# rpng/R-VIO

Measured on AMD Instinct MI355X. Metric: camera frames/sec (KLT+RANSAC track, IMU propagate, MSCKF update, augment/compose), 200 feat / 10-clone window, higher is better.
Workload: dtype f64 (filter) / u8+i32+f32 (KLT); 1 GPU; cfgB: synthetic EuRoC-shaped 752x480 @20Hz, 200 features, 10-clone window, IMU 200 Hz, single stream, equalizer on (CLAHE 3.0, 5x5), corners from the device detector (GFTT + cornerSubPix); parallelism=single GPU

## Files before the change

### r-vio_amd/csrc/filter_kernels.hip

```cpp
#include <type_traits>
#include "rvio_dev.h"
#include "../../include/rvio_hip.h"
#include "solve9.hip"

#include "literal.h"
__device__ const double kChi2Dev[500] = {
#include "chi2_table.inc"
};

typedef double d4 __attribute__((ext_vector_type(4)));

__device__ __forceinline__ double fast_rcp(double v) {
    double y = __builtin_amdgcn_rcp(v);
    y = fma(fma(-v, y, 1.0), y, y);
    return fma(fma(-v, y, 1.0), y, y);
}
__device__ __forceinline__ void sincos_fast(double x, double* sp, double* cp) {
    if (!(fabs(x) < 1e5)) { sincos(x, sp, cp); return; }
    const double kf = rint(x * 6.36619772367581382433e-01);
    double r = fma(-kf, 1.57079632679489655800e+00, x);
    r = fma(-kf, 6.12323399573676603587e-17, r);
    const int q = (int)kf & 3;
    const double z = r * r;
    double ps = fma(z, 1.58969099521155010221e-10, -2.50507602534068634195e-08);
// ... 1739 lines not shown
#pragma unroll
        for (int q = 0; q < 4; ++q) out[q] = p1[q] - acc[q] + s2 * acc2[q];
        return out;
    };
    const d4 xij = xtile(I * 16, J * 16);
    d4 xji = xij;
    if (I != J) xji = xtile(J * 16, I * 16);
#pragma unroll
    for (int q = 0; q < 4; ++q) tl[wave][lk + 4 * q][li] = xji[q];
    __builtin_amdgcn_wave_barrier();
#pragma unroll
    for (int q = 0; q < 4; ++q) {
        const int rr = lk + 4 * q, row = I * 16 + rr, col = J * 16 + li;
        const double v = .5 * (xij[q] + tl[wave][li][rr]);
        if (row < d && col < d) {
            Pout[(size_t)row + (size_t)col * ld] = v;
            if (I != J) Pout[(size_t)col + (size_t)row * ld] = v;
        }
    }
}

#define JL_LS 61
#define JL_LDS_DOUBLES (3 * 60 * JL_LS + 8 * 16 * JL_LS + 16)
__global__ __launch_bounds__(256) void joseph_lds_kernel(DevCfg cfg, int n, const double* __restrict__ P, const double* __restrict__ W, const double* __restrict__ Ab,
                                                         double* __restrict__ Pout, FilterMeta* __restrict__ meta, const double* __restrict__ x, double* __restrict__ x_out,
                                                         const double* __restrict__ dx_scr, int n_pairs, int dx_nt) {
    if (dx_scr && (int)blockIdx.x >= n_pairs) {
        __shared__ S9DxLds dxl;
        s9_dx_role(cfg, meta, n, Ab, x, P, dx_scr, x_out, dx_nt, (int)blockIdx.x - n_pairs, dxl);
        return;
    }
    extern __shared__ __align__(16) double jl[];
    constexpr int LS = JL_LS;
    double* const Wl = jl;
    double* const Al = Wl + 60 * LS;
    double* const Ccl = Al + 60 * LS;
    double* const PcS = Ccl + 60 * LS;
    double* const Us = PcS + 2 * 16 * LS;
    double* const Gs = Us + 2 * 16 * LS;
    double* const Qs = Gs + 2 * 16 * LS;
    constexpr int SS = 16 * LS;
    const int c6 = 6 * n, d = 24 + c6, ldh = cfg.ldh, ld = cfg.dmax;
    const double s2 = cfg.sigma_im * cfg.sigma_im;
    const int tid = threadIdx.x, lane = tid & 63, wave = tid >> 6, li = lane & 15, lk = lane >> 4;
    DBG_R(blockIdx.x == 0, 3);
    const int nt = (d + 15) / 16;
    int I = 0, rem = blockIdx.x;
    while (rem >= nt - I) { rem -= nt - I; ++I; }
    const int J = I + rem;
    const int r0[2] = {I * 16, J * 16};
    auto r0of = [&](int sidx) { return sidx ? J * 16 : I * 16; };
    DBG_T(20);
    double p0[4] = {0, 0, 0, 0}, p0t[4] = {0, 0, 0, 0};
    if (wave == 0) {
#pragma unroll
// ... 105 lines not shown
        for (int q = 0; q < 4; ++q) {
            if (wave < nprod) xt[wave][lk + 4 * q][li] = pa[q];
            if (two) xt[wave + 4][lk + 4 * q][li] = pb[q];
        }
    }
    __syncthreads();
    DBG_T(25);
    if (wave == 0) {
        const int o = (I == J) ? 0 : 3;
#pragma unroll
        for (int q = 0; q < 4; ++q) {
            const int rr = lk + 4 * q, row = I * 16 + rr, col = J * 16 + li;
            const double p1 = p0[q] - xt[0][rr][li];
            const double xij = p1 - xt[1][rr][li] + s2 * xt[2][rr][li];
            const double p1t = p0t[q] - xt[o][li][rr];
            const double xji = p1t - xt[o + 1][li][rr] + s2 * xt[o + 2][li][rr];
            const double v = .5 * (xij + xji);
            if (row < d && col < d) {
                Pout[(size_t)row + (size_t)col * ld] = v;
                if (I != J) Pout[(size_t)col + (size_t)row * ld] = v;
            }
        }
    }
}
```

### r-vio_amd/csrc/filter_kernels2.hip

```cpp
#pragma once
#include "rvio_dev.h"
#include "solve9.hip"

__device__ __forceinline__ double skew_e(const double* v, int i, int j) {
    if (i == j) return 0.0;
    const double e = v[3 - i - j];
    return (j == (i + 1) % 3) ? -e : e;
}

struct Prop3Sample { double dR[9], up[3], uv[3], w[3], dt, Rk[9], vk[3], gk[3]; };

template <int PROP3_CH>
struct Prop3Lds {
    double Pl[24][25];
    double Psi[24][25];
    double PhiSx[2][PROP3_CH][9][25];
    double PsiC[9][25];
    double Nq[PROP3_CH][9][6];
    double Qd[PROP3_CH][6][6];
    double vxs[PROP3_CH][9];
    Prop3Sample sm[PROP3_CH];
    double xs[26];
    double chain[9 + 3 * 5 + 1];
};
// ... 259 lines not shown
__global__ __launch_bounds__(256) void feat_prop_kernel(DevCfg cfg, int n, double* x, double* P,
                                                        const int* n_feat_ptr, const unsigned char* types, const int* lens, const float* meas,
                                                        double* Gshare, int* nrows_out, int* acc_out, int* ndof_out, double* gamma_out,
                                                        double* pfinv_out, double* tm_global, BatchIn bin,
                                                        FilterMeta* meta, const rvio_imu* imu, int m, double* chol_scr, int chol_nt, int shard_rank, int shard_world,
                                                        double* lit_rows) {
    DBG_R(blockIdx.x == 0, 0);
    DBG_W(blockIdx.x == 0 && threadIdx.x == 0, 28);
    extern __shared__ __align__(16) double fp_dyn[];
    if (blockIdx.x == gridDim.x - 1) { propagate_body<16>(cfg, meta, n, x, P, imu, m, 0, 0, *reinterpret_cast<Prop3Lds<16>*>(fp_dyn)); return; }
    if (chol_scr && blockIdx.x == gridDim.x - 2) {
        if (chol_nt == 4) s9_chol_role<2>(cfg, n, P, chol_scr, *reinterpret_cast<S9CholLds<4, 4>*>(fp_dyn));
        else s9_chol_role<3>(cfg, n, P, chol_scr, *reinterpret_cast<S9CholLds<6, 4>*>(fp_dyn));
        return;
    }
    feat_build_body<16>(cfg, n, x, P, n_feat_ptr, types, lens, meas, shard_rank, shard_world, Gshare, nrows_out, acc_out, ndof_out, gamma_out, pfinv_out, tm_global, 0, bin, meta, (int)blockIdx.x, nullptr, nullptr, lit_rows);
}

__device__ __forceinline__ int aug_src2(int a, int n, int nmax, int do_aug) {
    if (a < 24 || !do_aug) return a;
    const int cb = (a - 24) / 6, off = (a - 24) % 6;
    if (n < nmax) return (cb < n) ? a : 9 + off;
    return (cb < nmax - 1) ? a + 6 : 9 + off;
}
__global__ __launch_bounds__(256) void augcomp_kernel2(DevCfg cfg, int n, int do_aug, const double* __restrict__ x, const double* __restrict__ P,
                                                       double* __restrict__ x_out, double* __restrict__ P_out, double* __restrict__ pose_out, size_t bs,
                                                       unsigned long long* done) {
    DBG_R(blockIdx.x == 0, 5);
    x = zoff(x, bs); P = zoff(P, bs); x_out = zoff(x_out, bs); P_out = zoff(P_out, bs); pose_out = zoff(pose_out, bs);
    __shared__ double Vk[24][25];
    __shared__ double P11[24][25];
    __shared__ double Tm[24][25];
    __shared__ double xs[26];
    __shared__ double xo[17];
    const int nmax = cfg.nmax, ld = cfg.dmax;
    const int n2 = do_aug ? ((n < nmax) ? n + 1 : nmax) : n;
    const int d2 = 24 + 6 * n2, xd2 = 26 + 7 * n2;
    const int tid = threadIdx.x;
    if (tid < 26) xs[tid] = x[tid];
    for (int e = tid; e < 576; e += 256) Vk[e / 24][e % 24] = 0.0;
    const int gstride = ((int)gridDim.x - 1) * 256, e0 = ((int)blockIdx.x - 1) * 256 + tid, total = d2 * d2;
    double xv = 0.0, pr[9];
    bool pre = false;
    if (blockIdx.x == 0) {
        for (int e = tid; e < 576; e += 256) P11[e % 24][e / 24] = P[(size_t)(e % 24) + (size_t)(e / 24) * ld];
        static_assert(26 + 7 * (RVIO_MAX_LEN - 1) <= 256, "the state copy is one value per thread");
// ... 5 lines not shown
                else src = (cb < nmax - 1) ? i + 7 : 10 + off;
            }
            xv = x[src];
        }
    } else {
        for (int e = e0; e < total; e += gstride) {
            const int a = e % d2, b = e / d2;
            if (a < 24 && b < 24) continue;
            if (a >= 24 && b >= 24) { P_out[(size_t)a + (size_t)b * ld] = P[(size_t)aug_src2(a, n, nmax, do_aug) + (size_t)aug_src2(b, n, nmax, do_aug) * ld]; continue; }
            const int i = (a < 24) ? a : b;
            const double* pc = P + (size_t)aug_src2((a < 24) ? b : a, n, nmax, do_aug) * ld;
            if (i >= 15) P_out[(size_t)a + (size_t)b * ld] = pc[i];
            else if (i >= 9) P_out[(size_t)a + (size_t)b * ld] = 0.0;
            else if (e == e0) {
                const int b3 = 3 * (i / 3);
                pr[0] = pc[b3]; pr[1] = pc[b3 + 1]; pr[2] = pc[b3 + 2];
#pragma unroll
                for (int k = 0; k < 6; ++k) pr[3 + k] = pc[9 + k];
                pre = true;
            }
        }
    }
    __syncthreads();
    if (tid < 64) {
        const q4 qG = ldq(xs), qk = ldq(xs + 10);
        const d3 pG = ld3(xs + 4), pk = ld3(xs + 14);
        const m33 Rk = q2r(qk);
        const d3 gk = unit3(mv33(Rk, ld3(xs + 7)));
        const d3 pkG = mv33(Rk, sub3(pG, pk));
        if (tid == 0) {
            const m33 spx = skew33(pkG), sgx = skew33(gk);
#pragma unroll
            for (int i = 0; i < 3; ++i)
#pragma unroll
                for (int j = 0; j < 3; ++j) {
                    Vk[i][j] = Rk.m[3 * i + j];           Vk[i][9 + j] = (i == j) ? 1.0 : 0.0;
                    Vk[3 + i][3 + j] = Rk.m[3 * i + j];   Vk[3 + i][9 + j] = spx.m[3 * i + j];   Vk[3 + i][12 + j] = -Rk.m[3 * i + j];
                    Vk[6 + i][6 + j] = Rk.m[3 * i + j];   Vk[6 + i][9 + j] = sgx.m[3 * i + j];
                }
#pragma unroll
            for (int i = 15; i < 24; ++i) Vk[i][i] = 1.0;
            if (blockIdx.x == 0) {
                const q4 qkG = qmul(qk, qG);
                stq(xo, qkG); st3(xo + 4, pkG); st3(xo + 7, gk);
                xo[10] = 0; xo[11] = 0; xo[12] = 0; xo[13] = 1; xo[14] = 0; xo[15] = 0; xo[16] = 0;
                const d3 pGk = mv33(tr33(q2r(qG)), sub3(pk, pG));
                st3(pose_out, pGk); stq(pose_out + 3, qkG);
            }
        }
    }
    __syncthreads();
    if (blockIdx.x == 0) {
        for (int e = tid; e < 576; e += 256) {
            const int i = e / 24, j = e % 24;
            double a = 0;
            if (i >= 15) a = P11[i][j];
            else if (i < 9) {
                const int b3 = 3 * (i / 3);
#pragma unroll
                for (int k = 0; k < 3; ++k) a += Vk[i][b3 + k] * P11[b3 + k][j];
#pragma unroll
                for (int k = 9; k < 15; ++k) a += Vk[i][k] * P11[k][j];
            }
            Tm[i][j] = a;
        }
        __syncthreads();
        for (int e = tid; e < 576; e += 256) {
            const int i = e / 24, j = e % 24;
            double a = 0;
            if (j >= 15) a = Tm[i][j];
            else if (j < 9) {
                const int b3 = 3 * (j / 3);
#pragma unroll
                for (int k = 0; k < 3; ++k) a += Tm[i][b3 + k] * Vk[j][b3 + k];
#pragma unroll
                for (int k = 9; k < 15; ++k) a += Tm[i][k] * Vk[j][k];
            }
            P11[i][j] = a;
        }
        __syncthreads();
        for (int e = tid; e < 576; e += 256) { int i = e / 24, j = e % 24; P_out[(size_t)i + (size_t)j * ld] = .5 * (P11[i][j] + P11[j][i]); }
        for (int i = tid; i < xd2; i += 256) x_out[i] = (i < 17) ? xo[i] : xv;
    } else {
        for (int e = e0; e < total; e += gstride) {
            const int a = e % d2, b = e / d2;
            if ((a < 24) == (b < 24)) continue;
            const int i = (a < 24) ? a : b;
            if (i >= 9) continue;
            const int b3 = 3 * (i / 3);
            if (!(pre && e == e0)) {
                const double* pc = P + (size_t)aug_src2((a < 24) ? b : a, n, nmax, do_aug) * ld;
                pr[0] = pc[b3]; pr[1] = pc[b3 + 1]; pr[2] = pc[b3 + 2];
#pragma unroll
                for (int k = 0; k < 6; ++k) pr[3 + k] = pc[9 + k];
            }
            double acc = Vk[i][b3] * pr[0] + Vk[i][b3 + 1] * pr[1] + Vk[i][b3 + 2] * pr[2];
            acc += Vk[i][9] * pr[3] + Vk[i][10] * pr[4] + Vk[i][11] * pr[5];
            if (b3 == 3) acc += Vk[i][12] * pr[6] + Vk[i][13] * pr[7] + Vk[i][14] * pr[8];
            P_out[(size_t)a + (size_t)b * ld] = acc;
        }
    }
    DBG_R(blockIdx.x == 0, 6);
    if (done) stage_signal(done);
}
```

### r-vio_amd/csrc/rvio_hip.hip

```cpp
#include <hip/hip_runtime.h>
#include <atomic>
#include <chrono>
#include <dlfcn.h>
#include <cmath>
#include <cstdio>
#include <cstdlib>
#include <cstring>
#include <map>
#include <mutex>
#include <string>
#include <vector>

#include "../../include/rvio_hip.h"
#include "rvio_dev.h"
#include "frontend_dev.h"
#include "filter_kernels.hip"
#include "filter_kernels2.hip"
#include "solve6.hip"
#include "solve7.hip"
#include "solve9.hip"
#include "landmarks.hip"
#pragma clang fp contract(off)
#include "frontend_kernels.hip"
#include "klt3.hip"
// ... 6 lines not shown
    rvio_config cfg;
    DevCfg dc;
    int device = 0;
    hipStream_t stream = nullptr;
    hipStream_t stream_t = nullptr;
    hipStream_t ts = nullptr;
    hipEvent_t evT[4] = {nullptr, nullptr, nullptr, nullptr};
    hipEvent_t evH[4] = {nullptr, nullptr, nullptr, nullptr};
    static const int kHand = 4;
    hipEvent_t evF[kHand] = {nullptr, nullptr, nullptr, nullptr}, evIn[2] = {nullptr, nullptr};
    long frame_no = 0;
    bool piped = false, in_frame = false;
    struct TrackOut { int* n_feat; unsigned char* types; int* len; float* meas; } tout[kHand];
    std::string err;
    FilterMeta* meta = nullptr;
    double* x[2] = {nullptr, nullptr};
    double* P[2] = {nullptr, nullptr};
    int cur = 0;
    int img_count = 0;
    int n_clones_host = 0;
    double *partial = nullptr, *block = nullptr, *Ab = nullptr, *Tbuf = nullptr, *W = nullptr, *Mg = nullptr, *U = nullptr, *G = nullptr,
           *Pt1 = nullptr, *tm_global = nullptr, *gamma = nullptr, *pfinv = nullptr;
    int *nrows = nullptr, *acc = nullptr, *ndof = nullptr, *gram_cnt = nullptr;
    double* gpose = nullptr;
    int* gvalid = nullptr;
    size_t trunc_lds = 0, gram_batch_lds = 0;
    double *lit_rows = nullptr, *lit_state = nullptr;
    bool lit_state_global = false;
    size_t lit_batch_lds = 0;
    const double* last_Ab = nullptr;
    int feat_threads = 64;
    size_t feat_lds = 0, fprop_lds = 0, ug_lds = 0, book_lds = 0, jb_lds = 0;
    int book_waves = 4;
    bool book_fused = true;
    int solve5_variant = 0;
    StageSync* stage_sync = nullptr;
    StageSync stage_tgt = {};
    const unsigned long long* klt_wait = nullptr; unsigned long long klt_target = 0;
    unsigned long long* pyr_signal = nullptr;
    int solve7_variant = 0;
    int solve9_nt = 0;
    double* S9scr = nullptr;
    bool chol_ready = false;
    float* eig_map = nullptr;
    size_t solve5_lds = 0, cholt_lds = 0;
    rvio_imu* d_imu = nullptr;
    double* gathered = nullptr;
    int gathered_world = 0;
    int imu_cap = RVIO_MAX_IMU;
    float* d_cand = nullptr;
    uint8_t* d_img = nullptr;
    static const int kIC = 3;
    DetDev dets[kIC] = {};
    int det_set_last = 0;
    bool det_ready = false, use_det = false;
    hipStream_t stream_l = nullptr;
    hipEvent_t evA = nullptr, evL = nullptr;
    bool dx_pending = false;
    bool chol_async = false;
    hipStream_t stream_d = nullptr;
    hipStream_t stream_c = nullptr;
    hipEvent_t evC[kIC] = {nullptr, nullptr, nullptr};
    int n_ic = 2;
    int ic = 0;
    hipStream_t side = nullptr;
    hipEvent_t evD0 = nullptr, evD1 = nullptr;
    uint8_t* hb_img[2] = {nullptr, nullptr};
    rvio_imu* hb_imu[kHand + 1] = {nullptr, nullptr, nullptr, nullptr, nullptr};
    hipEvent_t book_wait = nullptr;
    int fin_mode[kHand] = {0, 0, 0, 0};
    unsigned long long fin_target[kHand] = {0, 0, 0, 0}, book_target = 0;
    bool book_dev = false;
    bool handover_evt = false;
    bool last_ra = false;
    float* hb_cand[2] = {nullptr, nullptr};
    static const int kPin = 3;
    uint8_t* pin[kPin] = {nullptr, nullptr, nullptr};
    hipEvent_t evPin[kPin] = {nullptr, nullptr, nullptr}, evPin2[kPin] = {nullptr, nullptr, nullptr};
    size_t pin_img = 0, pin_imu = 0, pin_bytes = 0;
    uint8_t *d_eq = nullptr, *d_lut2[kIC] = {nullptr, nullptr, nullptr};
// ... 149 lines not shown
    d->block_x = c->block_x; d->block_y = c->block_y;
    d->grid_cols = (int)std::floor(c->width / c->block_x);
    d->grid_rows = (int)std::floor(c->height / c->block_y);
    d->off_x = (float)(int)(.5 * (c->width - d->grid_cols * c->block_x));
    d->off_y = (float)(int)(.5 * (c->height - d->grid_rows * c->block_y));
    d->max_per_block = (d->grid_cols * d->grid_rows > 0) ? (float)(int)((float)c->n_features / (d->grid_cols * d->grid_rows)) : 0.f;
    d->use_sampson = c->use_sampson;
    d->fisheye = c->fisheye ? 1 : 0;
    int w = c->width, hgt = c->height, lv = 1;
    for (int l = 1; l <= 3; ++l) { w = (w + 1) / 2; hgt = (hgt + 1) / 2; if (w <= 15 || hgt <= 15) break; lv++; }
    d->levels = lv;
}

static int alloc_filter_slab(rvio_hip* h, bool need_tm_global) {
    const DevCfg& d = h->dc;
    const size_t dm = d.dmax, PP = dm * dm, ldh = d.ldh;
    TrackerDev& t = h->t;
    DALLOC(h, h->meta, 1);
    for (int b = 0; b < 2; ++b) { DALLOC(h, h->x[b], (size_t)d.xdmax + 8); DALLOC(h, h->P[b], PP); }
    DALLOC(h, h->partial, (size_t)d.Fu * ldh * ldh);
    DALLOC(h, h->block, 2 * ldh * ldh);
    DALLOC(h, h->Ab, 2 * ldh * ldh);
    DALLOC(h, h->gram_cnt, 8);
    DALLOC(h, h->stage_sync, 1);
    DALLOC(h, h->Tbuf, ldh * ldh); DALLOC(h, h->W, ldh * ldh);
    DALLOC(h, h->U, dm * ldh); DALLOC(h, h->G, dm * ldh);
    DALLOC(h, h->Pt1, PP);
    DALLOC(h, h->gamma, d.Fu); DALLOC(h, h->pfinv, (size_t)3 * d.Fu);
    DALLOC(h, h->nrows, d.Fu); DALLOC(h, h->acc, d.Fu); DALLOC(h, h->ndof, d.Fu);
    DALLOC(h, h->d_imu, RVIO_MAX_IMU);
    DALLOC(h, h->d_info, 1); DALLOC(h, h->d_pose, 8);
    DALLOC(h, t.n_feat, 1); DALLOC(h, t.types, d.Fu); DALLOC(h, t.len, d.Fu); DALLOC(h, t.meas, (size_t)2 * d.Fu * d.max_len);
    if (need_tm_global) DALLOC(h, h->tm_global, (size_t)d.Fu * d.rho_max * ldh);
    static const bool no_lit = getenv("RVIO_NO_LITERAL") != nullptr;
    if (!no_lit && d.ldh <= 190 && d.nmax + 1 <= 40 && d.rho_max < 254 && lit_slab_doubles(d.ldh, d.rho_max) * sizeof(double) <= 144 * 1024) {
        DALLOC(h, h->lit_rows, lit_rows_doubles(d.ldh, d.rho_max));
        if (h->lit_state_global) DALLOC(h, h->lit_state, lit_state_doubles(d.ldh - 1));
    }
    if (h->batch > 1 && d.max_len <= GEOM4_ML) { DALLOC(h, h->gpose, (size_t)d.Fu * (d.max_len - 1) * 24); DALLOC(h, h->gvalid, d.Fu); }
    return RVIO_OK;
}

static int detector_alloc(rvio_hip* h);
static int detector_check(rvio_hip* h);
static int alloc_frontend_slab(rvio_hip* h) {
    const DevCfg& d = h->dc;
// ... 51 lines not shown
    return e && *e && std::strcmp(e, "0") != 0 && std::strcmp(e, "False") != 0 && std::strcmp(e, "false") != 0;
}
static bool no_device_polls() {
    static const bool v = (paranoid_bits() & PAR_NO_DEVPOLL) || profiler_serialises();
    return v;
}

static hipError_t lds_attr(const void* fn, int bytes) {
    static std::mutex mu;
    static std::map<const void*, int> limit;
    std::lock_guard<std::mutex> lk(mu);
    int& cur = limit[fn];
    if (bytes <= cur) return hipSuccess;
    const hipError_t e = hipFuncSetAttribute(fn, hipFuncAttributeMaxDynamicSharedMemorySize, bytes);
    if (e == hipSuccess) cur = bytes;
    return e;
}
static_assert(LP_S9CHOL4_BYTES == sizeof(S9CholLds<4, 4>), "launch_plan.h: solve9's LDS structs");
static_assert(LP_S9CHOL6_BYTES == sizeof(S9CholLds<6, 4>), "launch_plan.h: solve9's LDS structs");
static_assert(LP_S9SMALL_BYTES == sizeof(S9SmallLds), "launch_plan.h: solve9's LDS structs");
static_assert(LP_PROP3_BYTES == sizeof(Prop3Lds<16>), "launch_plan.h: propagate's LDS struct");
static_assert(LP_JB_TL_DOUBLES == JB_TL_DOUBLES && LP_UGL_BYTES == UGL_LDS_DOUBLES * sizeof(double) && LP_FNL_BYTES == FNL_LDS_DOUBLES * sizeof(double) &&
              LP_JL_BYTES == JL_LDS_DOUBLES * sizeof(double), "launch_plan.h: the Joseph-form kernels' LDS");
static const void* lp_kernel_fn(int k) {
    switch (k) {
        case LPK_FEAT_BUILD16: return (const void*)feat_build_kernel<16>;
        case LPK_FEAT_BUILD4: return (const void*)feat_build_kernel<4>;
        case LPK_GRAM_REDUCE: return (const void*)gram_reduce_kernel;
        case LPK_BLOCK_SUM: return (const void*)block_sum_kernel;
        case LPK_LIT_BATCH: return (const void*)lit_batch_kernel;
        case LPK_GEMM_T_LDS: return (const void*)gemm_T_lds_kernel;
        case LPK_GRAM_BATCH4: return (const void*)gram_reduce_batch_kernel<4>;
        case LPK_GRAM_BATCH6: return (const void*)gram_reduce_batch_kernel<6>;
        case LPK_FEAT_PROP: return (const void*)feat_prop_kernel;
        case LPK_BOOKKEEP_B: return (const void*)bookkeep_b_kernel;
        case LPK_RANSAC_BOOK: return (const void*)ransac_book_kernel;
        case LPK_SOLVE9_SMALL: return (const void*)solve9_small_kernel;
        case LPK_SOLVE6_1: return (const void*)solve6_kernel<1, 8, 8>;
        case LPK_SOLVE6_2: return (const void*)solve6_kernel<2, 12, 8>;
        case LPK_SOLVE6_3: return (const void*)solve6_kernel<2, 16, 8>;
        case LPK_JOSEPH_BATCH: return (const void*)joseph_batch_kernel;
        case LPK_UG: return (const void*)ug_kernel;
        case LPK_UG_LDS: return (const void*)ug_lds_kernel;
        case LPK_FINAL_LDS: return (const void*)final_lds_kernel;
        case LPK_JOSEPH_LDS: return (const void*)joseph_lds_kernel;
    }
// ... 434 lines not shown
        return;
    }
    if (h->solve7_variant == 4)
        hipLaunchKernelGGL((solve7_kernel<3, 16, 12>), gb, dim3(768), 0, h->stream, d, h->meta, n, Ab, xin, Pc, h->Tbuf, h->W, xout, h->slab_bytes);
    else if (h->solve5_variant == 1)
        hipLaunchKernelGGL((solve6_kernel<1, 8, 8>), gb, dim3(512), h->solve5_lds, h->stream, d, h->meta, n, h->Tbuf, Ab, xin, Pc, h->W, xout, h->slab_bytes);
    else if (h->solve5_variant == 2)
        hipLaunchKernelGGL((solve6_kernel<2, 12, 8>), gb, dim3(512), h->solve5_lds, h->stream, d, h->meta, n, h->Tbuf, Ab, xin, Pc, h->W, xout, h->slab_bytes);
    else if (h->solve5_variant == 3)
        hipLaunchKernelGGL((solve6_kernel<2, 16, 8>), gb, dim3(512), h->solve5_lds, h->stream, d, h->meta, n, h->Tbuf, Ab, xin, Pc, h->W, xout, h->slab_bytes);
}

static void launch_ug_final(rvio_hip* h, int n, const double* Ab, double* Pn, bool ug, bool fin) {
    const DevCfg& d = h->dc;
    const int c6 = 6 * n, dd = 24 + c6, B = h->batch;
    const size_t bs = h->slab_bytes;
    double* Pc = h->P[h->cur];
    const int nt = (dd + 15) / 16, npair = nt * (nt + 1) / 2;
    if (h->jb_lds && ug && fin) {
        hipLaunchKernelGGL(joseph_batch_kernel, dim3(1, 1, B), dim3(JB_THREADS), h->jb_lds, h->stream, d, n, Pc, h->W, Ab, Pn, bs);
    } else if (B == 1 && c6 <= 60 && ug && fin) {
        const bool dxr = h->dx_pending;
        h->dx_pending = false;
        hipLaunchKernelGGL(joseph_lds_kernel, dim3(npair + (dxr ? (dd + 23) / 24 : 0)), dim3(256), JL_LDS_DOUBLES * sizeof(double), h->stream, d, n, Pc, h->W, Ab, Pn,
                           h->meta, (const double*)h->x[h->cur], h->x[h->cur ^ 1], dxr ? (const double*)h->S9scr : (const double*)nullptr, npair, h->solve9_nt);
    } else if (B == 1 && c6 <= 64) {
        if (ug) hipLaunchKernelGGL(ug_lds_kernel, dim3(nt), dim3(256), UGL_LDS_DOUBLES * sizeof(double), h->stream, d, n, Pc, h->W, Ab, h->U, h->G, h->Pt1);
        if (fin) hipLaunchKernelGGL(final_lds_kernel, dim3((npair + 3) / 4), dim3(256), FNL_LDS_DOUBLES * sizeof(double), h->stream, d, n, h->Pt1, h->G, h->U, Pn);
    } else if (B == 1) {
        const int c6t = (c6 + 15) / 16;
        if (ug) {
            const bool dxr = h->dx_pending;
            h->dx_pending = false;
            const double* nod = nullptr;
            hipLaunchKernelGGL(ug_tile_kernel<0>, dim3((nt * c6t + 3) / 4 + (dxr ? (dd + 23) / 24 : 0)), dim3(256), 0, h->stream, d, n, Pc, h->W, Ab, h->U, h->G, h->Pt1,
                               h->meta, (const double*)h->x[h->cur], h->x[h->cur ^ 1], dxr ? (const double*)h->S9scr : nod, h->solve9_nt);
            hipLaunchKernelGGL(ug_tile_kernel<1>, dim3((nt * c6t + 3) / 4), dim3(256), 0, h->stream, d, n, Pc, h->W, Ab, h->U, h->G, h->Pt1, h->meta, nod, (double*)nullptr, nod, 0);
            hipLaunchKernelGGL(ug_tile_kernel<2>, dim3((nt * nt + 3) / 4), dim3(256), 0, h->stream, d, n, Pc, h->W, Ab, h->U, h->G, h->Pt1, h->meta, nod, (double*)nullptr, nod, 0);
        }
        if (fin) hipLaunchKernelGGL(final_tile_kernel, dim3(npair), dim3(256), 0, h->stream, d, n, h->Pt1, h->G, h->U, Pn);
    } else {
        if (ug) hipLaunchKernelGGL(ug_kernel, dim3((dd + 15) / 16, 1, B), dim3(256), h->ug_lds, h->stream, d, n, Pc, h->W, Ab, h->U, h->G, h->Pt1, bs);
        if (fin) hipLaunchKernelGGL(final_kernel, dim3((npair + 3) / 4, 1, B), dim3(256), 0, h->stream, d, n, h->Pt1, h->G, h->U, Pn, bs);
    }
}

static void launch_landmarks(rvio_hip* h, int n, const LmOut& out) {
    const int T = std::min(LM_MAX_T, 64 * ((h->dc.Fu + 63) / 64));
// ... 126 lines not shown
    SYNC_FRONT(h);
    HIPCHK(h, hipStreamSynchronize(h->stream));
    const size_t o = (size_t)instance * h->lm.bs;
    int cnt = 0;
    if (h->lm_frame >= 0) {
        HIPCHK(h, hipMemcpyAsync(&cnt, (char*)h->lm.count + o, sizeof cnt, hipMemcpyDeviceToHost, h->stream));
        HIPCHK(h, hipStreamSynchronize(h->stream));
        cnt = std::max(0, std::min(cnt, h->dc.Fu));
    }
    if (n) *n = cnt;
    if (frame) *frame = h->lm_frame;
    if (cnt > 0) {
        if (feat) HIPCHK(h, hipMemcpyAsync(feat, (char*)h->lm.feat + o, sizeof(int) * cnt, hipMemcpyDeviceToHost, h->stream));
        if (p_r) HIPCHK(h, hipMemcpyAsync(p_r, (char*)h->lm.p_r + o, sizeof(double) * 3 * cnt, hipMemcpyDeviceToHost, h->stream));
        if (p_world) HIPCHK(h, hipMemcpyAsync(p_world, (char*)h->lm.p_w + o, sizeof(double) * 3 * cnt, hipMemcpyDeviceToHost, h->stream));
        HIPCHK(h, hipStreamSynchronize(h->stream));
    }
    return RVIO_OK;
}
int rvio_hip_get_landmarks(rvio_hip* h, int32_t* n, int32_t* frame, int32_t* feat, double* p_r, double* p_world) {
    return rvio_hip_get_landmarks_at(h, 0, n, frame, feat, p_r, p_world);
}

static int augment_compose_dev(rvio_hip* h, int do_augment) {
    const DevCfg& d = h->dc;
    const int c = h->cur, o = c ^ 1;
    const int cg = 1 + (h->batch >= 128 ? 4 : std::max(1, std::min(64, (d.dmax * d.dmax + 255) / 256)));
    unsigned long long* done = nullptr;
    if (h->batch == 1) { done = &h->stage_sync->aug; h->stage_tgt.aug += (unsigned long long)cg; }
    if (h->chol_async) { HIPCHK(h, hipStreamWaitEvent(h->stream, h->evL, 0)); h->chol_async = false; }
    hipLaunchKernelGGL(augcomp_kernel2, dim3(cg, 1, h->batch), dim3(256), 0, h->stream, d, h->n_clones_host, do_augment, h->x[c], h->P[c], h->x[o], h->P[o], h->d_pose,
                       h->slab_bytes, done);
    HIPCHK(h, hipGetLastError());
    h->cur = o;
    h->chol_ready = false;
    if (do_augment && h->n_clones_host < d.nmax) h->n_clones_host++;
    if (h->solve9_nt >= 8 && h->stream_l && !profiler_serialises() && h->n_clones_host >= 1) {
        HIPCHK(h, hipEventRecord(h->evA, h->stream));
        HIPCHK(h, hipStreamWaitEvent(h->stream_l, h->evA, 0));
        if (h->solve9_nt == 8) hipLaunchKernelGGL((solve9_chol_kernel<2, 4>), dim3(1), dim3(1024), 0, h->stream_l, d, h->n_clones_host, h->P[h->cur], h->S9scr);
        else hipLaunchKernelGGL((solve9_chol_kernel<3, 4>), dim3(1), dim3(1024), 0, h->stream_l, d, h->n_clones_host, h->P[h->cur], h->S9scr);
        HIPCHK(h, hipEventRecord(h->evL, h->stream_l));
        h->chol_async = true;
    }
    return RVIO_OK;
}
int rvio_hip_augment_compose(rvio_hip* h, int do_augment) {
    if (!h) return RVIO_ERR_INVALID;
    HIPCHK(h, hipSetDevice(h->device));
    return augment_compose_dev(h, do_augment);
}

static int detector_check(rvio_hip* h) {
    const int cell1 = (int)std::nearbyint((double)h->cfg.min_dist);
    if (cell1 < 1) { h->err = "Tracker.nMinDist < 1 is not supported by the device detector"; return RVIO_ERR_UNSUPPORTED; }
    const int spw = (int)std::floor(.5 * h->cfg.min_dist);
    if (spw < 1 || spw > 63) { h->err = "device cornerSubPix takes half-windows 1..63 (2 <= Tracker.nMinDist < 128)"; return RVIO_ERR_UNSUPPORTED; }
    return RVIO_OK;
}
static int detector_alloc_set(rvio_hip* h, DetDev& q) {
    const DevCfg& d = h->dc;
    const int cell1 = (int)std::nearbyint((double)h->cfg.min_dist), cell2 = (int)std::nearbyint((double)(2.f * h->cfg.min_dist));
    const size_t npx = (size_t)d.W * d.H;
    q.W = d.W; q.H = d.H; q.F = d.F; q.min_dist = h->cfg.min_dist; q.quality = (double)h->cfg.qual_lvl;
    q.max_cells = ((d.W + cell1 - 1) / cell1) * ((d.H + cell1 - 1) / cell1);
    q.first = h->t.first;
    q.eig = nullptr;
    DALLOC(h, q.maxkey, 1); DALLOC(h, q.counters, 4); DALLOC(h, q.cell_cnt, (size_t)q.max_cells);
// ... 316 lines not shown

int rvio_hip_frame_plan(rvio_hip* h, int* do_update, int* do_augment) {
    if (!h) return RVIO_ERR_INVALID;
    h->img_count++;
    if (do_update) *do_update = (h->n_clones_host > h->cfg.min_track_len - 1) ? 1 : 0;
    if (do_augment) *do_augment = (h->img_count > 1) ? 1 : 0;
    return RVIO_OK;
}
int rvio_hip_propagate_dev(rvio_hip* h, const rvio_imu* d_imu, int m) {
    if (!h || (!d_imu && m > 0) || m < 0) return RVIO_ERR_INVALID;
    HIPCHK(h, hipSetDevice(h->device));
    return propagate_dev(h, d_imu, m);
}

static int wait_filter_done(rvio_hip* h, int b, hipStream_t stream) {
    if (h->fin_mode[b] == 0) HIPCHK(h, hipStreamWaitEvent(stream, h->evF[b], 0));
    else HIPCHK(h, hipStreamSynchronize(h->stream));
    return RVIO_OK;
}
static int frame_tail_dev(rvio_hip* h, const rvio_imu* d_imu, int m, bool propagated = false) {
    h->img_count++;
    int rc = propagated ? RVIO_OK : propagate_dev(h, d_imu, m);
    if (rc != RVIO_OK) return rc;
    if (h->n_clones_host > h->cfg.min_track_len - 1) {
        rc = rvio_hip_update_tracked(h);
        if (rc != RVIO_OK) return rc;
    }
    return augment_compose_dev(h, h->img_count > 1);
}
int rvio_hip_frame_tracks_dev(rvio_hip* h, const rvio_imu* d_imu, int imu_stride, int m, const int32_t* d_n_feat, const unsigned char* d_types,
                              const int32_t* d_len, const float* d_meas) {
    if (!h || (!d_imu && m > 0) || m < 0 || imu_stride < 0 || (imu_stride > 0 && imu_stride < m)) return RVIO_ERR_INVALID;
    if (!d_n_feat || !d_types || !d_len || !d_meas) return RVIO_ERR_INVALID;
    if (h->piped || h->in_frame) { h->err = "rvio_hip_frame_tracks_dev on a handle that runs the pipelined image path"; return RVIO_ERR_INVALID; }
    HIPCHK(h, hipSetDevice(h->device));
    const DevCfg& d = h->dc;
    h->img_count++;
    const bool upd = h->n_clones_host > h->cfg.min_track_len - 1;
    const bool overlap = upd && h->batch > 1 && !h->front_end;
    int rc;
    if (overlap) {
        HIPCHK(h, hipEventRecord(h->evD0, h->stream));
        HIPCHK(h, hipStreamWaitEvent(h->stream_t, h->evD0, 0));
        rc = propagate_dev(h, d_imu, m, (size_t)imu_stride * sizeof(rvio_imu), h->stream_t);
        HIPCHK(h, hipEventRecord(h->evD1, h->stream_t));
    } else rc = propagate_dev(h, d_imu, m, (size_t)imu_stride * sizeof(rvio_imu));
    if (rc != RVIO_OK) return rc;
    if (upd) {
        const TrackerDev t0 = h->t;
        const BatchIn b0 = h->bin;
        h->t.n_feat = const_cast<int*>(d_n_feat); h->t.types = const_cast<unsigned char*>(d_types);
// ... 564 lines not shown
```

Before: 11060 frames/s.

## Fuse augment/compose into Joseph update kernel via last-block tail

Runs the augment/compose step as a tail inside joseph_lds_kernel: the last block to finish, detected with an atomic counter, builds Vk, rotates the 24x24 core block, transforms the cross-covariance columns and copies the clone block. This drops a separate augcomp_kernel2 launch and its dependency gap on the single-stream update path. The cost is that the whole augment runs serially in one 256-thread block rather than spread over many blocks. The host tracks the fused state and adjusts the stage-sync target to match.

```diff
diff --git a/r-vio_amd/csrc/filter_kernels.hip b/r-vio_amd/csrc/filter_kernels.hip
--- a/r-vio_amd/csrc/filter_kernels.hip
+++ b/r-vio_amd/csrc/filter_kernels.hip
@@ -1785,15 +1785,25 @@
 
 #define JL_LS 61
 #define JL_LDS_DOUBLES (3 * 60 * JL_LS + 8 * 16 * JL_LS + 16)
+struct AugTail { int on, do_aug; double* x_dst; double* P_dst; double* pose_out; int* cnt; unsigned long long* done; };
+__device__ void augcomp_tail(const DevCfg& cfg, int n, int do_aug, const double* x, const double* P, double* x_out, double* P_out, double* pose_out, double* lds);
+__device__ __forceinline__ void joseph_aug_tail(const DevCfg& cfg, int n, const AugTail& aug, const double* Pout, const double* x_out, double* lds) {
+    if (!last_block_done(aug.cnt, (int)gridDim.x)) return;
+    DBG_R(true, 5);
+    augcomp_tail(cfg, n, aug.do_aug, x_out, Pout, aug.x_dst, aug.P_dst, aug.pose_out, lds);
+    DBG_R(true, 6);
+    stage_signal(aug.done);
+}
 __global__ __launch_bounds__(256) void joseph_lds_kernel(DevCfg cfg, int n, const double* __restrict__ P, const double* __restrict__ W, const double* __restrict__ Ab,
                                                          double* __restrict__ Pout, FilterMeta* __restrict__ meta, const double* __restrict__ x, double* __restrict__ x_out,
-                                                         const double* __restrict__ dx_scr, int n_pairs, int dx_nt) {
+                                                         const double* __restrict__ dx_scr, int n_pairs, int dx_nt, AugTail aug) {
+    extern __shared__ __align__(16) double jl[];
     if (dx_scr && (int)blockIdx.x >= n_pairs) {
         __shared__ S9DxLds dxl;
         s9_dx_role(cfg, meta, n, Ab, x, P, dx_scr, x_out, dx_nt, (int)blockIdx.x - n_pairs, dxl);
+        if (aug.on) joseph_aug_tail(cfg, n, aug, Pout, x_out, jl);
         return;
     }
-    extern __shared__ __align__(16) double jl[];
     constexpr int LS = JL_LS;
     double* const Wl = jl;
     double* const Al = Wl + 60 * LS;
@@ -1945,4 +1955,5 @@
             }
         }
     }
-}
+    if (aug.on) joseph_aug_tail(cfg, n, aug, Pout, x_out, jl);
+}
diff --git a/r-vio_amd/csrc/filter_kernels2.hip b/r-vio_amd/csrc/filter_kernels2.hip
--- a/r-vio_amd/csrc/filter_kernels2.hip
+++ b/r-vio_amd/csrc/filter_kernels2.hip
@@ -305,6 +305,64 @@
     const int cb = (a - 24) / 6, off = (a - 24) % 6;
     if (n < nmax) return (cb < n) ? a : 9 + off;
     return (cb < nmax - 1) ? a + 6 : 9 + off;
+}
+__device__ __forceinline__ void aug_build_vk(const double* xs, double (*Vk)[25], double* xo, double* pose_out, bool head) {
+    const q4 qG = ldq(xs), qk = ldq(xs + 10);
+    const d3 pG = ld3(xs + 4), pk = ld3(xs + 14);
+    const m33 Rk = q2r(qk);
+    const d3 gk = unit3(mv33(Rk, ld3(xs + 7)));
+    const d3 pkG = mv33(Rk, sub3(pG, pk));
+    if (threadIdx.x == 0) {
+        const m33 spx = skew33(pkG), sgx = skew33(gk);
+#pragma unroll
+        for (int i = 0; i < 3; ++i)
+#pragma unroll
+            for (int j = 0; j < 3; ++j) {
+                Vk[i][j] = Rk.m[3 * i + j];           Vk[i][9 + j] = (i == j) ? 1.0 : 0.0;
+                Vk[3 + i][3 + j] = Rk.m[3 * i + j];   Vk[3 + i][9 + j] = spx.m[3 * i + j];   Vk[3 + i][12 + j] = -Rk.m[3 * i + j];
+                Vk[6 + i][6 + j] = Rk.m[3 * i + j];   Vk[6 + i][9 + j] = sgx.m[3 * i + j];
+            }
+#pragma unroll
+        for (int i = 15; i < 24; ++i) Vk[i][i] = 1.0;
+        if (head) {
+            const q4 qkG = qmul(qk, qG);
+            stq(xo, qkG); st3(xo + 4, pkG); st3(xo + 7, gk);
+            xo[10] = 0; xo[11] = 0; xo[12] = 0; xo[13] = 1; xo[14] = 0; xo[15] = 0; xo[16] = 0;
+            const d3 pGk = mv33(tr33(q2r(qG)), sub3(pk, pG));
+            st3(pose_out, pGk); stq(pose_out + 3, qkG);
+        }
+    }
+}
+__device__ __forceinline__ double aug_tm(const double (*Vk)[25], const double (*P11)[25], int i, int j) {
+    double a = 0;
+    if (i >= 15) a = P11[i][j];
+    else if (i < 9) {
+        const int b3 = 3 * (i / 3);
+#pragma unroll
+        for (int k = 0; k < 3; ++k) a += Vk[i][b3 + k] * P11[b3 + k][j];
+#pragma unroll
+        for (int k = 9; k < 15; ++k) a += Vk[i][k] * P11[k][j];
+    }
+    return a;
+}
+__device__ __forceinline__ double aug_p11(const double (*Vk)[25], const double (*Tm)[25], int i, int j) {
+    double a = 0;
+    if (j >= 15) a = Tm[i][j];
+    else if (j < 9) {
+        const int b3 = 3 * (j / 3);
+#pragma unroll
+        for (int k = 0; k < 3; ++k) a += Tm[i][b3 + k] * Vk[j][b3 + k];
+#pragma unroll
+        for (int k = 9; k < 15; ++k) a += Tm[i][k] * Vk[j][k];
+    }
+    return a;
+}
+__device__ __forceinline__ double aug_cross(const double (*Vk)[25], int i, const double* pr) {
+    const int b3 = 3 * (i / 3);
+    double acc = Vk[i][b3] * pr[0] + Vk[i][b3 + 1] * pr[1] + Vk[i][b3 + 2] * pr[2];
+    acc += Vk[i][9] * pr[3] + Vk[i][10] * pr[4] + Vk[i][11] * pr[5];
+    if (b3 == 3) acc += Vk[i][12] * pr[6] + Vk[i][13] * pr[7] + Vk[i][14] * pr[8];
+    return acc;
 }
 __global__ __launch_bounds__(256) void augcomp_kernel2(DevCfg cfg, int n, int do_aug, const double* __restrict__ x, const double* __restrict__ P,
                                                        double* __restrict__ x_out, double* __restrict__ P_out, double* __restrict__ pose_out, size_t bs,
@@ -356,62 +414,12 @@
         }
     }
     __syncthreads();
-    if (tid < 64) {
-        const q4 qG = ldq(xs), qk = ldq(xs + 10);
-        const d3 pG = ld3(xs + 4), pk = ld3(xs + 14);
-        const m33 Rk = q2r(qk);
-        const d3 gk = unit3(mv33(Rk, ld3(xs + 7)));
-        const d3 pkG = mv33(Rk, sub3(pG, pk));
-        if (tid == 0) {
-            const m33 spx = skew33(pkG), sgx = skew33(gk);
-#pragma unroll
-            for (int i = 0; i < 3; ++i)
-#pragma unroll
-                for (int j = 0; j < 3; ++j) {
-                    Vk[i][j] = Rk.m[3 * i + j];           Vk[i][9 + j] = (i == j) ? 1.0 : 0.0;
-                    Vk[3 + i][3 + j] = Rk.m[3 * i + j];   Vk[3 + i][9 + j] = spx.m[3 * i + j];   Vk[3 + i][12 + j] = -Rk.m[3 * i + j];
-                    Vk[6 + i][6 + j] = Rk.m[3 * i + j];   Vk[6 + i][9 + j] = sgx.m[3 * i + j];
-                }
-#pragma unroll
-            for (int i = 15; i < 24; ++i) Vk[i][i] = 1.0;
-            if (blockIdx.x == 0) {
-                const q4 qkG = qmul(qk, qG);
-                stq(xo, qkG); st3(xo + 4, pkG); st3(xo + 7, gk);
-                xo[10] = 0; xo[11] = 0; xo[12] = 0; xo[13] = 1; xo[14] = 0; xo[15] = 0; xo[16] = 0;
-                const d3 pGk = mv33(tr33(q2r(qG)), sub3(pk, pG));
-                st3(pose_out, pGk); stq(pose_out + 3, qkG);
-            }
-        }
-    }
+    if (tid < 64) aug_build_vk(xs, Vk, xo, pose_out, blockIdx.x == 0);
     __syncthreads();
     if (blockIdx.x == 0) {
-        for (int e = tid; e < 576; e += 256) {
-            const int i = e / 24, j = e % 24;
-            double a = 0;
-            if (i >= 15) a = P11[i][j];
-            else if (i < 9) {
-                const int b3 = 3 * (i / 3);
-#pragma unroll
-                for (int k = 0; k < 3; ++k) a += Vk[i][b3 + k] * P11[b3 + k][j];
-#pragma unroll
-                for (int k = 9; k < 15; ++k) a += Vk[i][k] * P11[k][j];
-            }
-            Tm[i][j] = a;
-        }
-        __syncthreads();
-        for (int e = tid; e < 576; e += 256) {
-            const int i = e / 24, j = e % 24;
-            double a = 0;
-            if (j >= 15) a = Tm[i][j];
-            else if (j < 9) {
-                const int b3 = 3 * (j / 3);
-#pragma unroll
-                for (int k = 0; k < 3; ++k) a += Tm[i][b3 + k] * Vk[j][b3 + k];
-#pragma unroll
-                for (int k = 9; k < 15; ++k) a += Tm[i][k] * Vk[j][k];
-            }
-            P11[i][j] = a;
-        }
+        for (int e = tid; e < 576; e += 256) Tm[e / 24][e % 24] = aug_tm(Vk, P11, e / 24, e % 24);
+        __syncthreads();
+        for (int e = tid; e < 576; e += 256) P11[e / 24][e % 24] = aug_p11(Vk, Tm, e / 24, e % 24);
         __syncthreads();
         for (int e = tid; e < 576; e += 256) { int i = e / 24, j = e % 24; P_out[(size_t)i + (size_t)j * ld] = .5 * (P11[i][j] + P11[j][i]); }
         for (int i = tid; i < xd2; i += 256) x_out[i] = (i < 17) ? xo[i] : xv;
@@ -428,12 +436,86 @@
 #pragma unroll
                 for (int k = 0; k < 6; ++k) pr[3 + k] = pc[9 + k];
             }
-            double acc = Vk[i][b3] * pr[0] + Vk[i][b3 + 1] * pr[1] + Vk[i][b3 + 2] * pr[2];
-            acc += Vk[i][9] * pr[3] + Vk[i][10] * pr[4] + Vk[i][11] * pr[5];
-            if (b3 == 3) acc += Vk[i][12] * pr[6] + Vk[i][13] * pr[7] + Vk[i][14] * pr[8];
-            P_out[(size_t)a + (size_t)b * ld] = acc;
+            P_out[(size_t)a + (size_t)b * ld] = aug_cross(Vk, i, pr);
         }
     }
     DBG_R(blockIdx.x == 0, 6);
     if (done) stage_signal(done);
 }
+
+#define AUG_TAIL_U 8
+#define AUG_TAIL_LDS_DOUBLES(c2) (3 * 600 + 32 + 24 + 25 * (c2))
+__device__ __noinline__ void augcomp_tail(const DevCfg& cfg, int n, int do_aug, const double* x, const double* P, double* x_out, double* P_out, double* pose_out, double* lds) {
+    double (*const Vk)[25] = reinterpret_cast<double (*)[25]>(lds);
+    double (*const P11)[25] = reinterpret_cast<double (*)[25]>(lds + 600);
+    double (*const Tm)[25] = reinterpret_cast<double (*)[25]>(lds + 1200);
+    double* const xs = lds + 1800;
+    double* const xo = lds + 1832;
+    double (*const cross)[25] = reinterpret_cast<double (*)[25]>(lds + 1856);
+    const int nmax = cfg.nmax, ld = cfg.dmax;
+    const int n2 = do_aug ? ((n < nmax) ? n + 1 : nmax) : n;
+    const int c2 = 6 * n2, xd2 = 26 + 7 * n2, ncross = 24 * c2, nblock = c2 * c2;
+    const int tid = threadIdx.x;
+    constexpr int U = AUG_TAIL_U;
+    double xsv = 0.0, xv = 0.0, pv[3], cv[U];
+    if (tid < 26) xsv = ld_l2(x + tid);
+#pragma unroll
+    for (int u = 0; u < 3; ++u) { const int e = min(tid + u * 256, 575); pv[u] = ld_l2(P + (size_t)(e % 24) + (size_t)(e / 24) * ld); }
+    if (tid < xd2) {
+        int src = tid;
+        if (tid >= 26 && do_aug) {
+            const int cb = (tid - 26) / 7, off = (tid - 26) % 7;
+            if (n < nmax) src = (cb < n) ? tid : 10 + off;
+            else src = (cb < nmax - 1) ? tid + 7 : 10 + off;
+        }
+        xv = ld_l2(x + src);
+    }
+    for (int e0 = 0; e0 < ncross; e0 += U * 256) {
+#pragma unroll
+        for (int u = 0; u < U; ++u) { const int e = min(e0 + tid + u * 256, ncross - 1); cv[u] = ld_l2(P + (size_t)(e % 24) + (size_t)aug_src2(24 + e / 24, n, nmax, do_aug) * ld); }
+#pragma unroll
+        for (int u = 0; u < U; ++u) { const int e = e0 + tid + u * 256; if (e < ncross) cross[e / 24][e % 24] = cv[u]; }
+    }
+    if (tid < 26) xs[tid] = xsv;
+    for (int e = tid; e < 576; e += 256) Vk[e / 24][e % 24] = 0.0;
+#pragma unroll
+    for (int u = 0; u < 3; ++u) { const int e = tid + u * 256; if (e < 576) P11[e % 24][e / 24] = pv[u]; }
+    auto copy_round = [&](int e0) {
+#pragma unroll
+        for (int u = 0; u < U; ++u) {
+            const int e = min(e0 + tid + u * 256, nblock - 1), a = e % c2, b = e / c2;
+            cv[u] = ld_l2(P + (size_t)aug_src2(24 + a, n, nmax, do_aug) + (size_t)aug_src2(24 + b, n, nmax, do_aug) * ld);
+        }
+#pragma unroll
+        for (int u = 0; u < U; ++u) {
+            const int e = e0 + tid + u * 256, a = e % c2, b = e / c2;
+            if (e < nblock) P_out[(size_t)(24 + a) + (size_t)(24 + b) * ld] = cv[u];
+        }
+    };
+    if (nblock) copy_round(0);
+    __syncthreads();
+    if (tid < 64) aug_build_vk(xs, Vk, xo, pose_out, true);
+    for (int e0 = U * 256; e0 < nblock; e0 += U * 256) copy_round(e0);
+    __syncthreads();
+    for (int e = tid; e < 576; e += 256) Tm[e / 24][e % 24] = aug_tm(Vk, P11, e / 24, e % 24);
+    for (int e = tid; e < ncross; e += 256) {
+        const int i = e % 24, c = e / 24;
+        double v = 0.0;
+        if (i >= 15) v = cross[c][i];
+        else if (i < 9) {
+            const int b3 = 3 * (i / 3);
+            double pr[9];
+            pr[0] = cross[c][b3]; pr[1] = cross[c][b3 + 1]; pr[2] = cross[c][b3 + 2];
+#pragma unroll
+            for (int k = 0; k < 6; ++k) pr[3 + k] = cross[c][9 + k];
+            v = aug_cross(Vk, i, pr);
+        }
+        P_out[(size_t)i + (size_t)(24 + c) * ld] = v;
+        P_out[(size_t)(24 + c) + (size_t)i * ld] = v;
+    }
+    __syncthreads();
+    for (int e = tid; e < 576; e += 256) P11[e / 24][e % 24] = aug_p11(Vk, Tm, e / 24, e % 24);
+    __syncthreads();
+    for (int e = tid; e < 576; e += 256) { int i = e / 24, j = e % 24; P_out[(size_t)i + (size_t)j * ld] = .5 * (P11[i][j] + P11[j][i]); }
+    if (tid < xd2) x_out[tid] = (tid < 17) ? xo[tid] : xv;
+}
diff --git a/r-vio_amd/csrc/rvio_hip.hip b/r-vio_amd/csrc/rvio_hip.hip
--- a/r-vio_amd/csrc/rvio_hip.hip
+++ b/r-vio_amd/csrc/rvio_hip.hip
@@ -52,6 +52,7 @@
     double *partial = nullptr, *block = nullptr, *Ab = nullptr, *Tbuf = nullptr, *W = nullptr, *Mg = nullptr, *U = nullptr, *G = nullptr,
            *Pt1 = nullptr, *tm_global = nullptr, *gamma = nullptr, *pfinv = nullptr;
     int *nrows = nullptr, *acc = nullptr, *ndof = nullptr, *gram_cnt = nullptr;
+    int* jl_cnt = nullptr;
     double* gpose = nullptr;
     int* gvalid = nullptr;
     size_t trunc_lds = 0, gram_batch_lds = 0;
@@ -86,6 +87,8 @@
     bool det_ready = false, use_det = false;
     hipStream_t stream_l = nullptr;
     hipEvent_t evA = nullptr, evL = nullptr;
+    int aug_tail = -1;
+    bool aug_fused = false;
     bool dx_pending = false;
     bool chol_async = false;
     hipStream_t stream_d = nullptr;
@@ -281,6 +284,7 @@
     DALLOC(h, h->block, 2 * ldh * ldh);
     DALLOC(h, h->Ab, 2 * ldh * ldh);
     DALLOC(h, h->gram_cnt, 8);
+    DALLOC(h, h->jl_cnt, 8);
     DALLOC(h, h->stage_sync, 1);
     DALLOC(h, h->Tbuf, ldh * ldh); DALLOC(h, h->W, ldh * ldh);
     DALLOC(h, h->U, dm * ldh); DALLOC(h, h->G, dm * ldh);
@@ -378,6 +382,7 @@
 static_assert(LP_PROP3_BYTES == sizeof(Prop3Lds<16>), "launch_plan.h: propagate's LDS struct");
 static_assert(LP_JB_TL_DOUBLES == JB_TL_DOUBLES && LP_UGL_BYTES == UGL_LDS_DOUBLES * sizeof(double) && LP_FNL_BYTES == FNL_LDS_DOUBLES * sizeof(double) &&
               LP_JL_BYTES == JL_LDS_DOUBLES * sizeof(double), "launch_plan.h: the Joseph-form kernels' LDS");
+static_assert(AUG_TAIL_LDS_DOUBLES(6 * (60 / 6 + 1)) <= JL_LDS_DOUBLES, "the augment / compose tail lives in joseph_lds_kernel's dynamic LDS (6n <= 60: 6n' <= 66)");
 static const void* lp_kernel_fn(int k) {
     switch (k) {
         case LPK_FEAT_BUILD16: return (const void*)feat_build_kernel<16>;
@@ -858,8 +863,11 @@
     } else if (B == 1 && c6 <= 60 && ug && fin) {
         const bool dxr = h->dx_pending;
         h->dx_pending = false;
+        AugTail aug = {0, 0, nullptr, nullptr, nullptr, nullptr, nullptr};
+        if (h->aug_tail >= 0) { aug = AugTail{1, h->aug_tail, h->x[h->cur], Pc, h->d_pose, h->jl_cnt, &h->stage_sync->aug}; h->aug_fused = true; }
+        h->aug_tail = -1;
         hipLaunchKernelGGL(joseph_lds_kernel, dim3(npair + (dxr ? (dd + 23) / 24 : 0)), dim3(256), JL_LDS_DOUBLES * sizeof(double), h->stream, d, n, Pc, h->W, Ab, Pn,
-                           h->meta, (const double*)h->x[h->cur], h->x[h->cur ^ 1], dxr ? (const double*)h->S9scr : (const double*)nullptr, npair, h->solve9_nt);
+                           h->meta, (const double*)h->x[h->cur], h->x[h->cur ^ 1], dxr ? (const double*)h->S9scr : (const double*)nullptr, npair, h->solve9_nt, aug);
     } else if (B == 1 && c6 <= 64) {
         if (ug) hipLaunchKernelGGL(ug_lds_kernel, dim3(nt), dim3(256), UGL_LDS_DOUBLES * sizeof(double), h->stream, d, n, Pc, h->W, Ab, h->U, h->G, h->Pt1);
         if (fin) hipLaunchKernelGGL(final_lds_kernel, dim3((npair + 3) / 4), dim3(256), FNL_LDS_DOUBLES * sizeof(double), h->stream, d, n, h->Pt1, h->G, h->U, Pn);
@@ -1032,16 +1040,27 @@
     return rvio_hip_get_landmarks_at(h, 0, n, frame, feat, p_r, p_world);
 }
 
-static int augment_compose_dev(rvio_hip* h, int do_augment) {
+static int augment_compose_dev(rvio_hip* h, int do_augment, bool fused = false) {
     const DevCfg& d = h->dc;
     const int c = h->cur, o = c ^ 1;
     const int cg = 1 + (h->batch >= 128 ? 4 : std::max(1, std::min(64, (d.dmax * d.dmax + 255) / 256)));
     unsigned long long* done = nullptr;
-    if (h->batch == 1) { done = &h->stage_sync->aug; h->stage_tgt.aug += (unsigned long long)cg; }
-    if (h->chol_async) { HIPCHK(h, hipStreamWaitEvent(h->stream, h->evL, 0)); h->chol_async = false; }
-    hipLaunchKernelGGL(augcomp_kernel2, dim3(cg, 1, h->batch), dim3(256), 0, h->stream, d, h->n_clones_host, do_augment, h->x[c], h->P[c], h->x[o], h->P[o], h->d_pose,
-                       h->slab_bytes, done);
-    HIPCHK(h, hipGetLastError());
+    if (h->batch == 1) { done = &h->stage_sync->aug; h->stage_tgt.aug += fused ? 1ull : (unsigned long long)cg; }
+    int rc = RVIO_OK;
+    if (h->chol_async) {
+        const hipError_t e = hipStreamWaitEvent(h->stream, h->evL, 0);
+        if (e != hipSuccess) {
+            h->err = std::string("hipStreamWaitEvent(h->stream, h->evL, 0): ") + hipGetErrorString(e);
+            if (!fused) return RVIO_ERR_NO_DEVICE;
+            rc = RVIO_ERR_NO_DEVICE;
+        }
+        h->chol_async = false;
+    }
+    if (!fused) {
+        hipLaunchKernelGGL(augcomp_kernel2, dim3(cg, 1, h->batch), dim3(256), 0, h->stream, d, h->n_clones_host, do_augment, h->x[c], h->P[c], h->x[o], h->P[o], h->d_pose,
+                           h->slab_bytes, done);
+        HIPCHK(h, hipGetLastError());
+    }
     h->cur = o;
     h->chol_ready = false;
     if (do_augment && h->n_clones_host < d.nmax) h->n_clones_host++;
@@ -1053,7 +1072,7 @@
         HIPCHK(h, hipEventRecord(h->evL, h->stream_l));
         h->chol_async = true;
     }
-    return RVIO_OK;
+    return rc;
 }
 int rvio_hip_augment_compose(rvio_hip* h, int do_augment) {
     if (!h) return RVIO_ERR_INVALID;
@@ -1416,11 +1435,17 @@
     h->img_count++;
     int rc = propagated ? RVIO_OK : propagate_dev(h, d_imu, m);
     if (rc != RVIO_OK) return rc;
+    const int do_aug = h->img_count > 1;
+    h->aug_fused = false;
     if (h->n_clones_host > h->cfg.min_track_len - 1) {
+        h->aug_tail = (h->batch == 1 && !h->lm_on) ? do_aug : -1;
         rc = rvio_hip_update_tracked(h);
-        if (rc != RVIO_OK) return rc;
-    }
-    return augment_compose_dev(h, h->img_count > 1);
+        h->aug_tail = -1;
+        if (rc != RVIO_OK) { h->aug_fused = false; return rc; }
+    }
+    const bool fused = h->aug_fused;
+    h->aug_fused = false;
+    return augment_compose_dev(h, do_aug, fused);
 }
 int rvio_hip_frame_tracks_dev(rvio_hip* h, const rvio_imu* d_imu, int imu_stride, int m, const int32_t* d_n_feat, const unsigned char* d_types,
                               const int32_t* d_len, const float* d_meas) {
```

Result: slower. 10150 frames/s (-8.2%).
